# kolyangg/open-universe

Measured on AMD Instinct MI355X. Metric: sec-audio enhanced/sec/GPU + xRT, UNIVERSE++ 16 kHz 8 s clips @1/2/4/8 GPU, higher is better.
Workload: dtype f32 (conv operands split into f16 hi/lo: 3 f16 MFMA passes, f32 accumulation)

## Files before the change

### include/ouhip.h

```cpp
#ifndef OUHIP_H
#define OUHIP_H

#include <stddef.h>
#include <stdint.h>

#ifdef __cplusplus
extern "C" {
#endif

#define OUHIP_ABI_VERSION 10

int ou_abi_version(void);
const char* ou_last_error(void);

typedef struct ou_conv_desc {
    const float* x;
    int64_t x_bstride;
    int64_t x_cstride;
    int32_t cin;
    int32_t in_len;
    int32_t frame;
    int32_t shift;
    const float* in_scale;
    float slope;
    const float* w;
    int32_t m;
    int32_t kt;
    int32_t pad;
    int32_t cc;
    int32_t n_frames;
    int32_t batch;
    float* y;
    int64_t y_bstride, y_cstride;
    int32_t rout;
    int32_t out_len;
    int32_t valid_len;
    const float* bias;
    const float* res1;
    int64_t r1_bstride, r1_cstride;
    float s1;
    const float* film;
    int64_t film_bstride;
    const float* res2;
    int64_t r2_bstride, r2_cstride;
    float s2;
    int32_t tile;
    int32_t prec;
    float w_unscale;
    int32_t f0;
    int32_t* status;
    float* ks_ws;
    int64_t ks_ws_bytes;
    uint16_t* sy;
    int64_t sy_bstride;
    int32_t sy_rows;
    int32_t sy_shift;
    float sy_slope;
    int32_t sy_pad_;
    const uint16_t* xs;
    int64_t xs_bstride;
    int32_t xs_rows;
    int32_t xs_shift;
    int32_t fir;
    int32_t fir_pad_;
    const float* fir_taps;
} ou_conv_desc;

int ou_conv_chunk(int kt, int frame);
int64_t ou_conv_packed_size(int m, int cin_eff, int kt, int cc);
int ou_conv_pack(const float* w_logical, int m, int cin_eff, int kt, int cc,
                 float* packed);
int ou_conv_pack_split(const float* w_logical, int m, int cin_eff, int kt,
                       float* packed, float* w_unscale);
int ou_conv_pack_split_nat(const float* w_logical, int m, int cin_eff, int kt,
                           float* packed, float* w_unscale);
int ou_conv(const ou_conv_desc* d, void* stream);
int ou_conv_pick_tile(const ou_conv_desc* d);
int ou_conv_num_tiles(void);
int ou_conv_tile_ok(int kt, int tile);
int ou_conv_lds_info(int kt, int tile, int* lds_request, int* device_optin_max);

typedef struct ou_gru_desc {
    const float* gi;
    int64_t gi_bstride;
    const float* w_hh;
    const float* b_hh;
    float* y;
    int64_t y_bstride, y_cstride;
    const float* res;
    int64_t res_bstride, res_cstride;
    float res_scale;
    int32_t hidden;
    int32_t steps;
    int32_t batch;
    int32_t flags;
    uint64_t* granules;
    int32_t* status;
    int32_t t_begin, t_end;
    float* hstate;
    int32_t ws_zeroed;
    int32_t _pad;
} ou_gru_desc;

int64_t ou_gru_workspace_bytes(int hidden, int batch);
int ou_gru(const ou_gru_desc* d, void* stream);

typedef struct ou_embed_desc {
    const float* sigma;
    int32_t n;
    int32_t kind;
    int32_t dim;
    float te_weight, te_bias;
    const float* rff_freq;
    int32_t n_rff;
    int32_t rows;
    const float* mlp_w[3];
    const float* mlp_b[3];
    float mlp_slope[3];
    const float* w;
    const float* bias;
    float* out;
    float* gbuf;
} ou_embed_desc;

int ou_embed(const ou_embed_desc* d, void* stream);

typedef struct ou_head_desc {
    const float* h;
    int64_t h_bstride;
    int32_t channels, length, batch, mode;
    float slope1, slope2;
    const float* w;
    float bias;
    int32_t edm, _pad;
    float w_skip, w_out, s2, c_score, c_noise, s_next;
    const float* x;
    const float* z;
    float* out;
} ou_head_desc;

int ou_head(const ou_head_desc* d, void* stream);

int ou_normalize(const float* x, float* y, int batch, int64_t n, float level,
                 float eps, void* stream);
int ou_inv_rms(const float* x, float* out, int batch, int64_t n, float denom,
               float eps, void* stream);
int ou_rms(const float* x, float* out, int batch, int64_t n, void* stream);
int ou_power(const float* x, float* y, int batch, int nf, int frames, void* stream);
int ou_pad(const float* x, int64_t x_bstride, float* y, int batch, int n_in,
           int n_out, int left, void* stream);
int ou_scale(const float* z, float* y, int64_t n, float scale, const float* add,
             void* stream);
int ou_finish(const float* x, int64_t x_bstride, int left, float* y, int batch,
              int len, const float* mix_rms, void* stream);
int ou_ensemble_reduce(const float* x, float* y, int ensemble, int64_t n,
                       int mode , void* stream);
int ou_signal_median(const float* x, float* y, int ensemble, int batch, int64_t n, int* counts,
                     void* stream);

int ou_resample(const float* x, int64_t x_bstride, float* y, int64_t y_bstride, int batch, int n_in,
                int n_out, const float* kernel, int phases, int taps, int orig, int width, void* stream);

int ou_flac_info(const uint8_t* data, int64_t n, int32_t* sample_rate, int32_t* channels,
                 int32_t* bits_per_sample, int64_t* frames);
int64_t ou_flac_decode(const uint8_t* data, int64_t n, float* out, int64_t frames);
int64_t ou_flac_encode_bound(int channels, int64_t frames, int bps);
int64_t ou_flac_encode(const float* x, int channels, int64_t frames, int sample_rate, int bps, uint8_t* out,
                       int64_t capacity);

typedef struct ou_snake_desc {
    const float* h;
    int64_t h_bstride;
    int32_t channels, length, batch, _pad0;
    const float* alpha;
    const float* k_up;
    int32_t taps_up, width_up;
    const float* k_down;
    int32_t taps_down, width_down;
    float* out;
} ou_snake_desc;

int ou_snake_aa(const ou_snake_desc* d, void* stream);

typedef struct ou_block_desc {
    const float* h;
    int64_t h_bstride, h_cstride;
    int32_t channels, length;
    int32_t batch, prec;
    const void* w[3];
    const float* bias[3];
    float slope[3];
    float w_unscale[3];
    const float* sc;
    int64_t sc_bstride, sc_cstride;
    float s_sc;
    int32_t dbg;
    const float* film;
    int64_t film_bstride;
    float* cond_out;
    int64_t co_bstride, co_cstride;
    float* y;
    int64_t y_bstride, y_cstride;
    float s_res, s2;
    const float* res2;
    int64_t r2_bstride, r2_cstride;
    int32_t* status;
    const float* x;
    int64_t x_bstride;
    const float* in_scale;
    const float* w_in;
    const float* b_in;
    ou_head_desc head;
    const void* w_down;
    const float* b_down;
    float slope_down, w_down_unscale;
    int32_t rate, down_kt;
    float* e;
    int64_t e_bstride, e_cstride;
    int32_t f0, f1;
    int32_t h0, h1;
    int32_t shift[4];
    uint16_t* sy;
    int64_t sy_bstride;
    int32_t sy_rows, sy_shift;
    float sy_slope;
    int32_t sy_pad_;
    const uint16_t* xs;
    int64_t xs_bstride;
    int32_t xs_rows, xs_pad_;
} ou_block_desc;

int ou_block_supported(int channels, int prec);
int ou_block_frames(int channels);
int64_t ou_block_packed_halves(int channels, int kt);
int ou_block_pack(const float* w, int channels, int kt, void* out, float* w_unscale);
int ou_block_pack_rect(const float* w, int m, int channels, int kt, void* out, float* w_unscale);
int64_t ou_block_packed_f32(int channels, int kt);
int ou_block_pack_f32(const float* w, int channels, int kt, float* out, float* w_unscale);
int ou_block_down_supported(int channels, int rate, int kt, int prec);
int ou_block(const ou_block_desc* d, void* stream);

typedef struct ou_program ou_program;

enum {
    OU_OP_CONV = 1, OU_OP_GRU = 2, OU_OP_EMBED = 3, OU_OP_HEAD = 4,
    OU_OP_NORMALIZE = 5, OU_OP_INV_RMS = 6, OU_OP_POWER = 7, OU_OP_PAD = 8,
    OU_OP_SCALE = 9, OU_OP_FINISH = 10, OU_OP_RMS = 11, OU_OP_SNAKE = 12,
    OU_OP_MEMSET = 13, OU_OP_ENSEMBLE = 14, OU_OP_BLOCK = 15,
    OU_OP_LANE = 16, OU_OP_SIGNAL = 17, OU_OP_WAIT = 18
};

typedef struct ou_memset_desc {
    void* ptr;
    int64_t bytes;
} ou_memset_desc;
typedef struct ou_norm_args {
    const float* x;
// ... 123 lines not shown
```

### open_universe_amd/_lib.py

```python
import ctypes
import os
from ctypes import POINTER, c_char, c_char_p, c_float, c_int, c_int32, c_int64, c_size_t, c_uint32, c_uint64, c_void_p

_HERE = os.path.dirname(os.path.abspath(__file__))
LIB_PATH = os.environ.get("OUHIP_LIB", os.path.join(_HERE, "libouhip.so"))
ABI_VERSION = 10

fp = c_void_p

OP_CONV, OP_GRU, OP_EMBED, OP_HEAD = 1, 2, 3, 4
OP_NORMALIZE, OP_INV_RMS, OP_POWER, OP_PAD = 5, 6, 7, 8
OP_SCALE, OP_FINISH, OP_RMS, OP_SNAKE = 9, 10, 11, 12
OP_MEMSET, OP_ENSEMBLE, OP_BLOCK = 13, 14, 15
OP_LANE, OP_SIGNAL, OP_WAIT = 16, 17, 18


class ConvDesc(ctypes.Structure):
    _fields_ = [
        ("x", fp), ("x_bstride", c_int64), ("x_cstride", c_int64),
        ("cin", c_int32), ("in_len", c_int32), ("frame", c_int32), ("shift", c_int32),
        ("in_scale", fp), ("slope", c_float), ("w", fp),
        ("m", c_int32), ("kt", c_int32), ("pad", c_int32), ("cc", c_int32),
        ("n_frames", c_int32), ("batch", c_int32),
        ("y", fp), ("y_bstride", c_int64), ("y_cstride", c_int64),
# ... 3 lines not shown
        ("film", fp), ("film_bstride", c_int64),
        ("res2", fp), ("r2_bstride", c_int64), ("r2_cstride", c_int64), ("s2", c_float),
        ("tile", c_int32), ("prec", c_int32), ("w_unscale", c_float), ("f0", c_int32),
        ("status", fp), ("ks_ws", fp), ("ks_ws_bytes", c_int64),
        ("sy", fp), ("sy_bstride", c_int64), ("sy_rows", c_int32), ("sy_shift", c_int32),
        ("sy_slope", c_float), ("sy_pad_", c_int32),
        ("xs", fp), ("xs_bstride", c_int64), ("xs_rows", c_int32), ("xs_shift", c_int32),
        ("fir", c_int32), ("fir_pad_", c_int32), ("fir_taps", fp),
    ]


class GruDesc(ctypes.Structure):
    _fields_ = [
        ("gi", fp), ("gi_bstride", c_int64), ("w_hh", fp), ("b_hh", fp),
        ("y", fp), ("y_bstride", c_int64), ("y_cstride", c_int64),
        ("res", fp), ("res_bstride", c_int64), ("res_cstride", c_int64),
        ("res_scale", c_float), ("hidden", c_int32), ("steps", c_int32), ("batch", c_int32),
        ("flags", c_int32), ("granules", fp), ("status", fp), ("t_begin", c_int32), ("t_end", c_int32),
        ("hstate", fp), ("ws_zeroed", c_int32), ("_pad", c_int32),
    ]


class EmbedDesc(ctypes.Structure):
    _fields_ = [
        ("sigma", fp), ("n", c_int32), ("kind", c_int32), ("dim", c_int32),
        ("te_weight", c_float), ("te_bias", c_float), ("rff_freq", fp), ("n_rff", c_int32),
        ("rows", c_int32), ("mlp_w", fp * 3), ("mlp_b", fp * 3), ("mlp_slope", c_float * 3),
        ("w", fp), ("bias", fp), ("out", fp), ("gbuf", fp),
    ]


class HeadDesc(ctypes.Structure):
    _fields_ = [
        ("h", fp), ("h_bstride", c_int64),
        ("channels", c_int32), ("length", c_int32), ("batch", c_int32), ("mode", c_int32),
        ("slope1", c_float), ("slope2", c_float), ("w", fp), ("bias", c_float),
        ("edm", c_int32), ("_pad", c_int32),
        ("w_skip", c_float), ("w_out", c_float), ("s2", c_float), ("c_score", c_float),
        ("c_noise", c_float), ("s_next", c_float),
        ("x", fp), ("z", fp), ("out", fp),
    ]


class SnakeDesc(ctypes.Structure):
    _fields_ = [
        ("h", fp), ("h_bstride", c_int64),
        ("channels", c_int32), ("length", c_int32), ("batch", c_int32), ("_pad0", c_int32),
        ("alpha", fp), ("k_up", fp), ("taps_up", c_int32), ("width_up", c_int32),
        ("k_down", fp), ("taps_down", c_int32), ("width_down", c_int32), ("out", fp),
    ]


class SyncArgs(ctypes.Structure):
    _fields_ = [("id", c_int32), ("_pad", c_int32)]


class MemsetArgs(ctypes.Structure):
    _fields_ = [("ptr", fp), ("bytes", c_int64)]


class NormArgs(ctypes.Structure):
    _fields_ = [("x", fp), ("y", fp), ("batch", c_int32), ("_pad", c_int32), ("n", c_int64),
                ("level", c_float), ("eps", c_float)]


class RmsArgs(ctypes.Structure):
    _fields_ = [("x", fp), ("out", fp), ("batch", c_int32), ("_pad", c_int32), ("n", c_int64),
                ("denom", c_float), ("eps", c_float)]


class PowerArgs(ctypes.Structure):
    _fields_ = [("x", fp), ("y", fp), ("batch", c_int32), ("nf", c_int32),
                ("frames", c_int32), ("_pad", c_int32)]


class PadArgs(ctypes.Structure):
    _fields_ = [("x", fp), ("x_bstride", c_int64), ("y", fp), ("batch", c_int32),
                ("n_in", c_int32), ("n_out", c_int32), ("left", c_int32)]


class ScaleArgs(ctypes.Structure):
    _fields_ = [("z", fp), ("y", fp), ("n", c_int64), ("scale", c_float), ("_pad", c_float),
                ("add", fp)]


class FinishArgs(ctypes.Structure):
    _fields_ = [("x", fp), ("x_bstride", c_int64), ("left", c_int32), ("batch", c_int32),
                ("len", c_int32), ("_pad", c_int32), ("y", fp), ("mix_rms", fp)]


class EnsembleArgs(ctypes.Structure):
    _fields_ = [("x", fp), ("y", fp), ("ensemble", c_int32), ("mode", c_int32), ("n", c_int64),
                ("batch", c_int32), ("_pad", c_int32), ("counts", c_void_p)]


class BlockDesc(ctypes.Structure):
    _fields_ = [
        ("h", fp), ("h_bstride", c_int64), ("h_cstride", c_int64),
        ("channels", c_int32), ("length", c_int32), ("batch", c_int32), ("prec", c_int32),
        ("w", fp * 3), ("bias", fp * 3), ("slope", c_float * 3), ("w_unscale", c_float * 3),
        ("sc", fp), ("sc_bstride", c_int64), ("sc_cstride", c_int64), ("s_sc", c_float), ("dbg", c_int32),
        ("film", fp), ("film_bstride", c_int64),
        ("cond_out", fp), ("co_bstride", c_int64), ("co_cstride", c_int64),
        ("y", fp), ("y_bstride", c_int64), ("y_cstride", c_int64), ("s_res", c_float), ("s2", c_float),
        ("res2", fp), ("r2_bstride", c_int64), ("r2_cstride", c_int64),
        ("status", fp),
        ("x", fp), ("x_bstride", c_int64), ("in_scale", fp), ("w_in", fp), ("b_in", fp),
        ("head", HeadDesc),
        ("w_down", fp), ("b_down", fp), ("slope_down", c_float), ("w_down_unscale", c_float),
        ("rate", c_int32), ("down_kt", c_int32), ("e", fp), ("e_bstride", c_int64), ("e_cstride", c_int64),
        ("f0", c_int32), ("f1", c_int32), ("h0", c_int32), ("h1", c_int32),
        ("shift", c_int32 * 4),
        ("sy", fp), ("sy_bstride", c_int64), ("sy_rows", c_int32), ("sy_shift", c_int32),
        ("sy_slope", c_float), ("sy_pad_", c_int32),
        ("xs", fp), ("xs_bstride", c_int64), ("xs_rows", c_int32), ("xs_pad_", c_int32),
    ]


class BundleIo(ctypes.Structure):
    _fields_ = [("region", c_int32), ("count", c_int32), ("offset", c_int64),
                ("batch", c_int32), ("length", c_int32)]


class BundleMeta(ctypes.Structure):
    _fields_ = [("mix", BundleIo), ("noise", BundleIo), ("out", BundleIo), ("status", BundleIo),
                ("n_regions", c_int32), ("n_ops", c_int32), ("region_bytes", c_int64),
                ("json", c_char_p), ("json_bytes", c_int64), ("arch", c_char * 16)]


OP_STRUCT = {
    OP_CONV: ConvDesc, OP_GRU: GruDesc, OP_EMBED: EmbedDesc, OP_HEAD: HeadDesc,
    OP_NORMALIZE: NormArgs, OP_INV_RMS: RmsArgs, OP_RMS: RmsArgs, OP_POWER: PowerArgs,
    OP_PAD: PadArgs, OP_SCALE: ScaleArgs, OP_FINISH: FinishArgs, OP_SNAKE: SnakeDesc,
    OP_MEMSET: MemsetArgs, OP_ENSEMBLE: EnsembleArgs, OP_BLOCK: BlockDesc,
    OP_LANE: SyncArgs, OP_SIGNAL: SyncArgs, OP_WAIT: SyncArgs,
}

EXPORTS = {
    "ou_abi_version": (c_int, []),
    "ou_last_error": (ctypes.c_char_p, []),
    "ou_conv_chunk": (c_int, [c_int, c_int]),
    "ou_conv_packed_size": (c_int64, [c_int, c_int, c_int, c_int]),
    "ou_conv_pack": (c_int, [POINTER(c_float), c_int, c_int, c_int, c_int, POINTER(c_float)]),
    "ou_conv_pack_split": (c_int, [POINTER(c_float), c_int, c_int, c_int, POINTER(c_float),
                                   POINTER(c_float)]),
    "ou_conv_pack_split_nat": (c_int, [POINTER(c_float), c_int, c_int, c_int, POINTER(c_float),
                                       POINTER(c_float)]),
    "ou_conv": (c_int, [POINTER(ConvDesc), c_void_p]),
    "ou_conv_pick_tile": (c_int, [POINTER(ConvDesc)]),
    "ou_conv_num_tiles": (c_int, []),
    "ou_conv_tile_ok": (c_int, [c_int, c_int]),
    "ou_conv_lds_info": (c_int, [c_int, c_int, POINTER(c_int), POINTER(c_int)]),
    "ou_gru_workspace_bytes": (c_int64, [c_int, c_int]),
    "ou_gru": (c_int, [POINTER(GruDesc), c_void_p]),
    "ou_embed": (c_int, [POINTER(EmbedDesc), c_void_p]),
    "ou_head": (c_int, [POINTER(HeadDesc), c_void_p]),
    "ou_normalize": (c_int, [fp, fp, c_int, c_int64, c_float, c_float, c_void_p]),
    "ou_inv_rms": (c_int, [fp, fp, c_int, c_int64, c_float, c_float, c_void_p]),
    "ou_rms": (c_int, [fp, fp, c_int, c_int64, c_void_p]),
    "ou_power": (c_int, [fp, fp, c_int, c_int, c_int, c_void_p]),
    "ou_pad": (c_int, [fp, c_int64, fp, c_int, c_int, c_int, c_int, c_void_p]),
    "ou_scale": (c_int, [fp, fp, c_int64, c_float, fp, c_void_p]),
    "ou_finish": (c_int, [fp, c_int64, c_int, fp, c_int, c_int, fp, c_void_p]),
    "ou_ensemble_reduce": (c_int, [fp, fp, c_int, c_int64, c_int, c_void_p]),
    "ou_signal_median": (c_int, [fp, fp, c_int, c_int, c_int64, c_void_p, c_void_p]),
    "ou_snake_aa": (c_int, [POINTER(SnakeDesc), c_void_p]),
    "ou_block_supported": (c_int, [c_int, c_int]),
    "ou_block_frames": (c_int, [c_int]),
    "ou_block_packed_halves": (c_int64, [c_int, c_int]),
    "ou_block_pack": (c_int, [POINTER(c_float), c_int, c_int, c_void_p, POINTER(c_float)]),
    "ou_block_packed_f32": (c_int64, [c_int, c_int]),
    "ou_block_pack_f32": (c_int, [POINTER(c_float), c_int, c_int, POINTER(c_float), POINTER(c_float)]),
    "ou_block_pack_rect": (c_int, [POINTER(c_float), c_int, c_int, c_int, c_void_p, POINTER(c_float)]),
    "ou_block_down_supported": (c_int, [c_int, c_int, c_int, c_int]),
    "ou_block": (c_int, [POINTER(BlockDesc), c_void_p]),
    "ou_resample": (c_int, [fp, c_int64, fp, c_int64, c_int, c_int, c_int, fp, c_int, c_int, c_int, c_int,
                            c_void_p]),
    "ou_flac_info": (c_int, [c_void_p, c_int64, POINTER(c_int32), POINTER(c_int32), POINTER(c_int32),
                             POINTER(c_int64)]),
    "ou_flac_decode": (c_int64, [c_void_p, c_int64, c_void_p, c_int64]),
    "ou_flac_encode_bound": (c_int64, [c_int, c_int64, c_int]),
    "ou_flac_encode": (c_int64, [c_void_p, c_int, c_int64, c_int, c_int, c_void_p, c_int64]),
    "ou_program_create": (c_void_p, []),
    "ou_program_destroy": (None, [c_void_p]),
    "ou_program_add": (c_int, [c_void_p, c_int, c_void_p, c_size_t]),
    "ou_program_patch": (c_int, [c_void_p, c_int, c_int, c_void_p, c_size_t]),
    "ou_program_size": (c_int, [c_void_p]),
    "ou_program_run": (c_int, [c_void_p, c_void_p]),
    "ou_program_capture": (c_int, [c_void_p]),
    "ou_program_capture_segments": (c_int, [c_void_p]),
    "ou_program_validate": (c_int, [c_void_p]),
    "ou_program_launch": (c_int, [c_void_p, c_void_p]),
    "ou_program_op_kind": (c_int, [c_void_p, c_int]),
    "ou_program_profile": (c_int, [c_void_p, c_void_p, POINTER(c_float)]),
    "ou_program_trace": (c_int, [c_void_p, c_void_p, POINTER(c_float), POINTER(c_float)]),
    "ou_randn": (c_int, [fp, c_int64, c_uint64, c_uint64, c_void_p]),
    "ou_philox4x32": (c_int, [POINTER(c_uint32), POINTER(c_uint32), POINTER(c_uint32)]),
    "ou_bundle_open": (c_int, [c_char_p, POINTER(c_void_p)]),
    "ou_bundle_close": (None, [c_void_p]),
    "ou_bundle_info": (c_int, [c_void_p, POINTER(BundleMeta)]),
    "ou_bundle_region": (c_int, [c_void_p, c_int, POINTER(c_int32), POINTER(c_int64), POINTER(c_void_p)]),
    "ou_bundle_op": (c_int, [c_void_p, c_int, POINTER(c_int32), POINTER(c_int64), POINTER(c_char_p)]),
    "ou_bundle_materialize": (c_int, [c_void_p, POINTER(c_uint64), c_int, c_void_p]),
    "ou_bundle_load": (c_int, [c_char_p, c_int, POINTER(c_void_p)]),
    "ou_model_enhance_noise": (c_int, [c_void_p, fp, fp, fp, c_void_p]),
    "ou_model_enhance": (c_int, [c_void_p, fp, fp, c_uint64, c_uint64, c_void_p]),
    "ou_model_status": (c_int, [c_void_p]),
    "ou_model_info": (c_int, [c_void_p, POINTER(BundleMeta)]),
    "ou_model_destroy": (None, [c_void_p]),
    "ou_long_windows": (c_int, [c_int64, c_int, c_int, POINTER(c_int64), POINTER(c_int64)]),
    "ou_long_fade": (c_int, [c_int, POINTER(c_float)]),
    "ou_window_gather": (c_int, [fp, c_int64, c_int, c_int64, c_int, c_int, c_int64, c_int, c_int64, fp, c_int64,
                                 c_int64, c_void_p]),
    "ou_overlap_add": (c_int, [fp, c_int64, c_int64, c_int, c_int, c_int64, c_int, fp, fp, c_void_p]),
    "ou_model_long_noise": (c_int64, [c_void_p, c_int64, c_int, POINTER(c_int64)]),
    "ou_model_enhance_long_noise": (c_int, [c_void_p, fp, c_int64, c_int, fp, fp, c_void_p]),
    "ou_model_enhance_long": (c_int, [c_void_p, fp, c_int64, c_int, fp, c_uint64, c_uint64, fp, c_void_p]),
}

_lib = None


class OuHipError(RuntimeError):
    pass


class OuRangeError(OuHipError):
    flags = ()


def load():
    global _lib
    if _lib is not None:
        return _lib
    if not os.path.exists(LIB_PATH):
        raise OuHipError(
            f"{LIB_PATH} not found: build it with `python -c 'import __graft_entry__ as g; "
            "g.build()'` or open_universe_amd/csrc/build.sh")
    lib = ctypes.CDLL(LIB_PATH)
    for name, (res, args) in EXPORTS.items():
        f = getattr(lib, name)
        f.restype = res
        f.argtypes = args
    if lib.ou_abi_version() != ABI_VERSION:
        raise OuHipError("libouhip ABI version mismatch")
    _lib = lib
    return lib


def check(rc, what=""):
    if rc != 0:
        msg = load().ou_last_error()
        raise OuHipError(f"{what}: ouhip error {rc}: {msg.decode() if msg else ''}")


def conv_chunk(kt, frame):
    return load().ou_conv_chunk(kt, frame)


def conv_pack(w_logical, cc):
    import numpy as np

    w = np.ascontiguousarray(w_logical, dtype=np.float32)
    m, cin, kt = w.shape
    n = load().ou_conv_packed_size(m, cin, kt, cc)
    out = np.empty(n, dtype=np.float32)
    check(load().ou_conv_pack(w.ctypes.data_as(POINTER(c_float)), m, cin, kt, cc,
                              out.ctypes.data_as(POINTER(c_float))), "conv_pack")
    return out


def _split_scale(w):
    import numpy as np

    if not np.isfinite(w).all():
        raise OuHipError("split packing: non-finite weight")
    mx = float(np.abs(w).max()) if w.size else 0.0
    e = 0
    if mx > 0.0:
        e = min(100, max(-100, 10 - int(np.frexp(np.float32(mx))[1])))
    return np.float32(2.0**e), float(2.0 ** (6 - e))


def _hi_lo(a):
    import numpy as np

    hi = a.astype(np.float16)
    lo = ((a - hi.astype(np.float32)) * np.float32(2048.0)).astype(np.float16)
    return hi, lo


def conv_pack_split_np(w_logical):
    import numpy as np

    w = np.ascontiguousarray(w_logical, dtype=np.float32)
    m, cin, kt = w.shape
    sc, unscale = _split_scale(w)
    mt = (m + 31) // 32
    cpad = (cin + 63) // 64 * 64
    a = np.zeros((mt * 32, cpad, kt), dtype=np.float32)
    a[:m, :cin] = w * sc
    a = a.reshape(mt, 32, cpad // 16, 8, 2, kt).transpose(0, 2, 5, 4, 1, 3)
    hi, lo = _hi_lo(np.ascontiguousarray(a))
    out = np.stack([hi, lo], axis=2)
    return np.ascontiguousarray(out).reshape(-1).view(np.float32), unscale

# ... 218 lines not shown
```

### open_universe_amd/csrc/ou_gru.hip

```cpp
#include <hip/hip_runtime.h>

#include "../../include/ouhip.h"
#include "ou_common.h"

namespace {

constexpr int kMaxBatchPerWG = 4;

__host__ __device__ constexpr int64_t xcc_slot_base(int batch, int hidden) { return (int64_t)batch * 4 * hidden; }
__host__ __device__ constexpr int64_t xcc_slot_count(int batch, int hidden) { return (int64_t)batch * hidden / 4; }

#ifdef OU_GRU_STAMPS
constexpr int kStampSlots = 8;
#define OU_STAMP_INIT uint64_t st_[5] = {0, 0, 0, 0, 0}; uint64_t tp_ = __builtin_amdgcn_s_memtime();
#define OU_STAMP(i) do { const uint64_t n_ = __builtin_amdgcn_s_memtime(); st_[i] += n_ - tp_; tp_ = n_; } while (0)
#else
constexpr int kStampSlots = 0;
#define OU_STAMP_INIT
#define OU_STAMP(i) do { } while (0)
#endif

__device__ __forceinline__ float sigmoidf_(float x) { return 1.0f / (1.0f + expf(-x)); }

#define OU_DPP(v, ctrl) __builtin_bit_cast(float, __builtin_amdgcn_mov_dpp(__builtin_bit_cast(int, (v)), (ctrl), 0xF, 0xF, true))
__device__ __forceinline__ float sum8(float v)
{
    v += OU_DPP(v, 0xB1);
    v += OU_DPP(v, 0x4E);
    v += OU_DPP(v, 0x141);
    return v;
}

template <int H, int NB, int U>
__global__ __launch_bounds__(8 * U) void gru_kernel(ou_gru_desc d, int nb, int nchains, int flags)
{
    constexpr int G = H / U;
    constexpr int NT = 8 * U;
    constexpr int KPL = H / 8;
    constexpr int SEG = KPL + 4;
    __shared__ __attribute__((aligned(16))) float hs[NB][8 * SEG];
    __shared__ int abort_flag;

    const int bid = blockIdx.x;
    int chain, member;
    if (flags & 1) {
        const int c8 = bid & 7, rest = bid >> 3;
        member = rest % G;
        chain = (rest / G) * 8 + ((c8 - (flags >> 12)) & 7);
    } else {
        chain = bid / G;
        member = bid % G;
    }
    if (chain >= nchains) return;
    const int dir = chain & 1;
    const int b0 = (chain >> 1) * nb;

    const int tid = threadIdx.x;
    const int lane = tid & 63;
    const int wave = tid >> 6;
    const int kg = lane & 7;
    const int u = lane >> 3;
    const int j = member * U + wave * 8 + u;
    const int nbh = min(nb, d.batch - b0);
    const int T = d.steps;
    const bool sleep_poll = !(flags & 2);
    const bool nowait = flags & 16;
    if (tid == 0) abort_flag = 0;

    const float* wbase = d.w_hh + (int64_t)dir * 3 * H * H;
    float wr[KPL], wz[KPL], wn[KPL];
#pragma unroll
    for (int k = 0; k < KPL; k += 4) {
        const float4 a = *(const float4*)(wbase + (int64_t)(0 * H + j) * H + kg * KPL + k);
        const float4 bq = *(const float4*)(wbase + (int64_t)(1 * H + j) * H + kg * KPL + k);
        const float4 c = *(const float4*)(wbase + (int64_t)(2 * H + j) * H + kg * KPL + k);
        wr[k] = a.x; wr[k + 1] = a.y; wr[k + 2] = a.z; wr[k + 3] = a.w;
        wz[k] = bq.x; wz[k + 1] = bq.y; wz[k + 2] = bq.z; wz[k + 3] = bq.w;
        wn[k] = c.x; wn[k + 1] = c.y; wn[k + 2] = c.z; wn[k + 3] = c.w;
    }
    const float bhr = d.b_hh[dir * 3 * H + 0 * H + j];
    const float bhz = d.b_hh[dir * 3 * H + 1 * H + j];
    const float bhn = d.b_hh[dir * 3 * H + 2 * H + j];

    uint64_t* gran = d.granules;
    auto gidx = [&](int b, int par, int k) -> int64_t {
        return (((int64_t)b * 2 + dir) * 2 + par) * H + k;
    };

    float gir[NB], giz[NB], gin[NB], rsd[NB];
    auto prefetch = [&](int step, float* pr, float* pz, float* pn, float* pres) {
        const int tm = dir == 0 ? step : T - 1 - step;
#pragma unroll
        for (int bb = 0; bb < NB; ++bb) {
            if (bb < nbh && kg == 0) {
                const float* g = d.gi + (int64_t)(b0 + bb) * d.gi_bstride +
                                 (int64_t)(dir * 3 * H) * T + tm;
                pr[bb] = g[(int64_t)(0 * H + j) * T];
                pz[bb] = g[(int64_t)(1 * H + j) * T];
                pn[bb] = g[(int64_t)(2 * H + j) * T];
                pres[bb] = d.res ? d.res[(int64_t)(b0 + bb) * d.res_bstride +
                                         (int64_t)(dir * H + j) * d.res_cstride + tm]
                                 : 0.f;
            }
        }
    };
    prefetch(0, gir, giz, gin, rsd);
    OU_STAMP_INIT

    for (int t = 0; t < T; ++t) {
        const int time = dir == 0 ? t : T - 1 - t;
        if (t == 0) {
            for (int i = tid; i < nbh * H; i += NT) {
                const int bb = i / H, k = i - bb * H;
                hs[bb][(k / KPL) * SEG + (k % KPL)] = 0.f;
            }
        } else {
            const uint32_t want = (uint32_t)t;
            const int par = (t - 1) & 1;
            constexpr int NPER = (NB * H + NT - 1) / NT;
            uint64_t v[NPER];
            uint64_t* pp[NPER];
#pragma unroll
            for (int e = 0; e < NPER; ++e) {
                const int i = tid + e * NT;
                const int bb = i / H, k = i - bb * H;
                pp[e] = gran + gidx(b0 + min(bb, nbh - 1), par, k);
                v[e] = (i < nbh * H) ? __hip_atomic_load(pp[e], __ATOMIC_RELAXED, __HIP_MEMORY_SCOPE_AGENT)
                                     : ((uint64_t)want << 32);
            }
            uint32_t spins = 0;
            while (true) {
                bool ok = true;
                if (nowait) break;
#pragma unroll
                for (int e = 0; e < NPER; ++e) ok &= (uint32_t)(v[e] >> 32) == want;
                if (ok) break;
                if (sleep_poll) __builtin_amdgcn_s_sleep(1);
                if (++spins > (1u << 23)) {
                    atomicExch(d.status, 1);
                    abort_flag = 1;
                    break;
                }
#pragma unroll
                for (int e = 0; e < NPER; ++e)
                    if ((uint32_t)(v[e] >> 32) != want)
                        v[e] = __hip_atomic_load(pp[e], __ATOMIC_RELAXED, __HIP_MEMORY_SCOPE_AGENT);
            }
            OU_STAMP(0);
#pragma unroll
            for (int e = 0; e < NPER; ++e) {
                const int i = tid + e * NT;
                if (i < nbh * H) {
                    const int bb = i / H, k = i - bb * H;
                    hs[bb][(k / KPL) * SEG + (k % KPL)] = __uint_as_float((uint32_t)v[e]);
                }
            }
        }
        __syncthreads();
        if (abort_flag) return;
        OU_STAMP(1);

        float cr[NB], cz[NB], cn[NB], cres[NB];
#pragma unroll
        for (int bb = 0; bb < NB; ++bb) {
            cr[bb] = gir[bb]; cz[bb] = giz[bb]; cn[bb] = gin[bb]; cres[bb] = rsd[bb];
        }
        if (t + 1 < T) prefetch(t + 1, gir, giz, gin, rsd);

#pragma unroll
        for (int bb = 0; bb < NB; ++bb) {
            if (bb >= nbh) break;
            const float* hv = &hs[bb][kg * SEG];
            float sr = 0.f, sz = 0.f, sn = 0.f;
#pragma unroll
            for (int k = 0; k < KPL; k += 4) {
                const float4 hq = *(const float4*)(hv + k);
                sr = fmaf(wr[k], hq.x, sr); sz = fmaf(wz[k], hq.x, sz); sn = fmaf(wn[k], hq.x, sn);
                sr = fmaf(wr[k + 1], hq.y, sr); sz = fmaf(wz[k + 1], hq.y, sz); sn = fmaf(wn[k + 1], hq.y, sn);
                sr = fmaf(wr[k + 2], hq.z, sr); sz = fmaf(wz[k + 2], hq.z, sz); sn = fmaf(wn[k + 2], hq.z, sn);
                sr = fmaf(wr[k + 3], hq.w, sr); sz = fmaf(wz[k + 3], hq.w, sz); sn = fmaf(wn[k + 3], hq.w, sn);
            }
            sr = sum8(sr);
            sz = sum8(sz);
            sn = sum8(sn);
            OU_STAMP(2);
            if (kg == 0) {
                const float hprev = hs[bb][(j / KPL) * SEG + (j % KPL)];
                const float r = sigmoidf_(cr[bb] + (sr + bhr));
                const float z = sigmoidf_(cz[bb] + (sz + bhz));
                const float n = tanhf(cn[bb] + r * (sn + bhn));
                const float hn = (1.0f - z) * n + z * hprev;
                const int b = b0 + bb;
                if (t + 1 < T) {
                    const uint64_t g = ((uint64_t)(uint32_t)(t + 1) << 32) | __float_as_uint(hn);
                    __hip_atomic_store(gran + gidx(b, t & 1, j), g, __ATOMIC_RELAXED,
                                       __HIP_MEMORY_SCOPE_AGENT);
                }
                const int64_t c = (int64_t)(dir * H + j);
                const float out = d.res ? (hn + cres[bb]) * d.res_scale : hn;
                d.y[(int64_t)b * d.y_bstride + c * d.y_cstride + time] = out;
            }
        }
        OU_STAMP(3);
        __syncthreads();
        OU_STAMP(4);
    }
#ifdef OU_GRU_STAMPS
    if (tid == 0) {
        uint64_t* o = gran + xcc_slot_base(d.batch, H) + xcc_slot_count(d.batch, H) + (int64_t)bid * kStampSlots;
        for (int i = 0; i < 5; ++i) o[i] = st_[i];
        o[5] = T;
    }
#endif
}


__device__ __forceinline__ float fast_sigmoid(float x)
{
    return __builtin_amdgcn_rcpf(1.0f + __builtin_amdgcn_exp2f(-1.44269504088896341f * x));
}
__device__ __forceinline__ float fast_tanh(float x)
{
    return fmaf(2.0f, fast_sigmoid(2.0f * x), -1.0f);
}

__device__ __forceinline__ void swap32(float& x, float& y)
{
    const auto r = __builtin_amdgcn_permlane32_swap(__float_as_uint(x), __float_as_uint(y), false, false);
    x = __uint_as_float(r[0]);
    y = __uint_as_float(r[1]);
}
__device__ __forceinline__ void swap16(float& x, float& y)
{
    const auto r = __builtin_amdgcn_permlane16_swap(__float_as_uint(x), __float_as_uint(y), false, false);
    x = __uint_as_float(r[0]);
    y = __uint_as_float(r[1]);
}

constexpr int kKsWaves = 4;


template <int H, int NB, int UW>
__global__ __launch_bounds__(64 * kKsWaves) void gru_ks_kernel(ou_gru_desc d, int nb, int nchains, int flags,
                                                               int bofs)
{
    constexpr int KPL = H / 64;
    constexpr int G = H / (UW * kKsWaves);
    constexpr int NV = UW * 3 * NB;
    constexpr int NG = 3 * NB;
    constexpr int USH = UW == 8 ? 3 : 4;
    static_assert(H % 64 == 0 && G >= 1 && (UW == 4 || UW == 8), "k-split GRU: H % 64 == 0, UW 4 or 8");

    const int bid = blockIdx.x;
    int chain, member;
    if (flags & 1) {
        const int c8 = bid & 7, rest = bid >> 3;
        member = rest % G;
        chain = (rest / G) * 8 + ((c8 - (flags >> 12)) & 7);
    } else {
        chain = bid / G;
        member = bid % G;
    }
    if (chain >= nchains) return;
    const int dir = chain & 1;
    const int b0 = bofs + (chain >> 1) * nb;
    const int nbh = min(nb, d.batch - b0);
    const int T = d.steps;
    const bool sleep_poll = !(flags & 2);

    const int lane = threadIdx.x & 63;
    const int wave = threadIdx.x >> 6;
    const int ubase = (member * kKsWaves + wave) * UW;
    const int j = ubase + (lane >> USH);
    const bool writer = (lane & ((1 << USH) - 1)) == 0;

    float w[UW][3][KPL];
    const float* wbase = d.w_hh + (int64_t)dir * 3 * H * H + lane * KPL;
#pragma unroll
    for (int u = 0; u < UW; ++u)
#pragma unroll
        for (int g = 0; g < 3; ++g)
#pragma unroll
            for (int k = 0; k < KPL; ++k) w[u][g][k] = wbase[(int64_t)(g * H + ubase + u) * H + k];
    const float bhr = d.b_hh[dir * 3 * H + 0 * H + j];
    const float bhz = d.b_hh[dir * 3 * H + 1 * H + j];
    const float bhn = d.b_hh[dir * 3 * H + 2 * H + j];

    uint64_t* gran = d.granules;

    bool local_l2 = false;
    if (!(flags & 64)) {
        uint32_t xcc;
        asm volatile("s_getreg_b32 %0, hwreg(HW_REG_XCC_ID, 0, 4)" : "=s"(xcc));
        uint64_t* xs = gran + xcc_slot_base(d.batch, H) + ((int64_t)b0 * 2 + dir) * G;
        if (threadIdx.x == 0)
            __hip_atomic_store(xs + member, (1ull << 32) | xcc, __ATOMIC_RELAXED, __HIP_MEMORY_SCOPE_AGENT);
        uint64_t v = 0;
        for (uint32_t spins = 0;; ++spins) {
            v = lane < G ? __hip_atomic_load(xs + lane, __ATOMIC_RELAXED, __HIP_MEMORY_SCOPE_AGENT)
                         : ((1ull << 32) | xcc);
            if (__all((uint32_t)(v >> 32) == 1u)) break;
            if (spins > (1u << 23)) {
                if (lane == 0) atomicExch(d.status, 1);
                return;
            }
            __builtin_amdgcn_s_sleep(1);
        }
        local_l2 = __all((uint32_t)v == xcc);
    }
    const int64_t gran_bytes = (int64_t)d.batch * 2 * 2 * H * 8;
    const __amdgpu_buffer_rsrc_t grsrc =
        ou_rsrc(gran, gran_bytes);
    auto goff = [&](int b, int par) -> int {
        return (int)(((((int64_t)b * 2 + dir) * 2 + par) * H + lane * KPL) * 8);
    };

    const int tb = d.t_begin, te = d.t_end > 0 ? min(d.t_end, T) : T;
    float hp[NB];
    float gir[NB], giz[NB], gin[NB], rsd[NB];
    auto prefetch = [&](int step) {
        const int tm = dir == 0 ? step : T - 1 - step;
#pragma unroll
        for (int bb = 0; bb < NB; ++bb) {
            if (bb < nbh) {
                const float* g = d.gi + (int64_t)(b0 + bb) * d.gi_bstride + (int64_t)(dir * 3 * H) * T + tm;
                gir[bb] = g[(int64_t)(0 * H + j) * T];
                giz[bb] = g[(int64_t)(1 * H + j) * T];
                gin[bb] = g[(int64_t)(2 * H + j) * T];
                rsd[bb] = d.res ? d.res[(int64_t)(b0 + bb) * d.res_bstride +
                                        (int64_t)(dir * H + j) * d.res_cstride + tm]
                                : 0.f;
            }
        }
    };
    constexpr int CS = UW == 4 ? 128 : 64;
    const bool stage = NB == 1 && !(flags & 256);
    float4* gst = nullptr;
    if constexpr (NB == 1) {
        __shared__ float4 gst_all[kKsWaves][CS * UW];
        gst = gst_all[wave];
    }
    const int wv = __builtin_amdgcn_readfirstlane(wave);
    auto stage_chunk = [&](int c0) {
        constexpr int NV4 = 4 * UW * CS / 64;
        const int ub = (member * kKsWaves + wv) * UW;
        float v[NV4];
#pragma unroll
        for (int i = 0; i < NV4; ++i) {
            const int e = lane + 64 * i, row = e / CS, st = min(c0 + e % CS, te - 1);
            const int tm = dir == 0 ? st : T - 1 - st;
            if (row < 3 * UW) {
                const int g = row / UW, u = row % UW;
                v[i] = d.gi[(int64_t)b0 * d.gi_bstride + (int64_t)(dir * 3 * H + g * H + ub + u) * T + tm];
            } else {
                const int u = row - 3 * UW;
                v[i] = d.res ? d.res[(int64_t)b0 * d.res_bstride + (int64_t)(dir * H + ub + u) * d.res_cstride + tm]
                             : 0.f;
            }
        }
#pragma unroll
        for (int i = 0; i < NV4; ++i) {
            const int e = lane + 64 * i, row = e / CS, sc = e % CS;
            const int comp = row < 3 * UW ? row / UW : 3, u = row < 3 * UW ? row % UW : row - 3 * UW;
            ((float*)gst)[(sc * UW + u) * 4 + comp] = v[i];
        }
    };
    auto hs_at = [&](int b, int u) -> float {
        return tb > 0 ? d.hstate[((int64_t)b * 2 + dir) * H + u] : 0.f;
    };
    float h0[NB][KPL];
#pragma unroll
    for (int bb = 0; bb < NB; ++bb) {
        hp[bb] = hs_at(b0 + min(bb, nbh - 1), j);
#pragma unroll
        for (int k = 0; k < KPL; ++k) h0[bb][k] = hs_at(b0 + min(bb, nbh - 1), lane * KPL + k);
    }
    if (stage) stage_chunk(tb);
    else prefetch(tb);
    OU_STAMP_INIT

    for (int t = tb; t < te; ++t) {
        const int time = dir == 0 ? t : T - 1 - t;
        float h[NB][KPL];
        float4 gv{};
        if (stage) {
            if (t > tb && (t - tb) % CS == 0) stage_chunk(t);
            gv = gst[((t - tb) % CS) * UW + (lane >> USH)];
        }
        if (t == tb) {
#pragma unroll
            for (int bb = 0; bb < NB; ++bb)
#pragma unroll
                for (int k = 0; k < KPL; ++k) h[bb][k] = h0[bb][k];
        } else {
            const uint32_t want = (uint32_t)t;
            const int par = (t - 1) & 1;
            for (uint32_t spins = 0;; ++spins) {
                bool ok = true;
#pragma unroll
                for (int bb = 0; bb < NB; ++bb) {
                    const int b = b0 + min(bb, nbh - 1);
                    if constexpr (KPL % 2 == 0) {
#pragma unroll
                        for (int q = 0; q < KPL / 2; ++q) {
                            const auto v = __builtin_amdgcn_raw_buffer_load_b128(grsrc, goff(b, par) + 16 * q, 0, 16);
                            h[bb][2 * q] = __uint_as_float(v[0]);
                            h[bb][2 * q + 1] = __uint_as_float(v[2]);
                            ok &= bb >= nbh || (v[1] == want && v[3] == want);
                        }
                    } else {
#pragma unroll
                        for (int k = 0; k < KPL; ++k) {
                            const uint64_t v = __hip_atomic_load(
                                gran + ((((int64_t)b * 2 + dir) * 2 + par) * H + lane * KPL + k),
                                __ATOMIC_RELAXED, __HIP_MEMORY_SCOPE_AGENT);
                            h[bb][k] = __uint_as_float((uint32_t)v);
                            ok &= bb >= nbh || (uint32_t)(v >> 32) == want;
                        }
                    }
                }
                if (__all(ok)) break;
                if (sleep_poll) __builtin_amdgcn_s_sleep(1);
                if (spins > (1u << 23)) {
                    if (lane == 0) atomicExch(d.status, 1);
                    return;
                }
                asm volatile("" ::: "memory");
            }
        }
        OU_STAMP(0);

        float cr[NB], cz[NB], cn[NB], cres[NB];
        if (stage) {
            cr[0] = gv.x, cz[0] = gv.y, cn[0] = gv.z, cres[0] = gv.w;
        } else {
#pragma unroll
            for (int bb = 0; bb < NB; ++bb) {
                cr[bb] = gir[bb]; cz[bb] = giz[bb]; cn[bb] = gin[bb]; cres[bb] = rsd[bb];
            }
            if (t + 1 < te) prefetch(t + 1);
        }

        float acc[NV];
#pragma unroll
        for (int u = 0; u < UW; ++u)
#pragma unroll
            for (int bb = 0; bb < NB; ++bb)
#pragma unroll
                for (int g = 0; g < 3; ++g) {
                    float a = 0.f;
#pragma unroll
                    for (int k = 0; k < KPL; ++k) a = fmaf(w[u][g][k], h[bb][k], a);
                    acc[(u * NB + bb) * 3 + g] = a;
                }
        OU_STAMP(1);

#pragma unroll
        for (int i = 0; i < NV / 2; ++i) {
            swap32(acc[i], acc[i + NV / 2]);
            acc[i] += acc[i + NV / 2];
        }
#pragma unroll
        for (int i = 0; i < NV / 4; ++i) {
            swap16(acc[i], acc[i + NV / 4]);
            acc[i] += acc[i + NV / 4];
        }
        if constexpr (UW == 8) {
            const bool hi8 = lane & 8;
#pragma unroll
            for (int i = 0; i < NG; ++i) {
                const float send = hi8 ? acc[i] : acc[i + NG];
                const float keep = hi8 ? acc[i + NG] : acc[i];
                acc[i] = keep + OU_DPP(send, 0x128);
            }
        } else {
#pragma unroll
            for (int i = 0; i < NG; ++i) acc[i] += OU_DPP(acc[i], 0x128);
        }
#pragma unroll
        for (int i = 0; i < NG; ++i) acc[i] = sum8(acc[i]);
        OU_STAMP(2);

#pragma unroll
        for (int bb = 0; bb < NB; ++bb) {
            if (bb >= nbh) break;
            const float r = fast_sigmoid(cr[bb] + (acc[bb * 3 + 0] + bhr));
            const float z = fast_sigmoid(cz[bb] + (acc[bb * 3 + 1] + bhz));
            const float n = fast_tanh(cn[bb] + r * (acc[bb * 3 + 2] + bhn));
            const float hn = (1.0f - z) * n + z * hp[bb];
            hp[bb] = hn;
            if (writer) {
                const int b = b0 + bb;
                if (t + 1 < T) {
                    const uint64_t gv = ((uint64_t)(uint32_t)(t + 1) << 32) | __float_as_uint(hn);
                    uint64_t* gp = gran + ((((int64_t)b * 2 + dir) * 2 + (t & 1)) * H + j);
                    if (local_l2)
                        __hip_atomic_store(gp, gv, __ATOMIC_RELAXED, __HIP_MEMORY_SCOPE_WORKGROUP);
                    else
                        __hip_atomic_store(gp, gv, __ATOMIC_RELAXED, __HIP_MEMORY_SCOPE_AGENT);
                }
                const float out = d.res ? (hn + cres[bb]) * d.res_scale : hn;
                d.y[(int64_t)b * d.y_bstride + (int64_t)(dir * H + j) * d.y_cstride + time] = out;
            }
        }
        OU_STAMP(3);
    }
    if (d.hstate && writer) {
#pragma unroll
        for (int bb = 0; bb < NB; ++bb)
            if (bb < nbh) d.hstate[((int64_t)(b0 + bb) * 2 + dir) * H + j] = hp[bb];
    }
    if (!(flags & 64) && threadIdx.x == 0)
        __hip_atomic_store(gran + xcc_slot_base(d.batch, H) + ((int64_t)b0 * 2 + dir) * G + member, (uint64_t)0,
                           __ATOMIC_RELAXED, __HIP_MEMORY_SCOPE_AGENT);
#ifdef OU_GRU_STAMPS
    if (lane == 0 && wave == 0) {
        uint64_t* o = gran + xcc_slot_base(d.batch, H) + xcc_slot_count(d.batch, H) + (int64_t)bid * kStampSlots;
        for (int i = 0; i < 4; ++i) o[i] = st_[i];
        o[4] = local_l2;
        o[5] = T;
    }
#endif
}

template <int H, int NB, int UW>
void launch_ks(const ou_gru_desc& d, int nb, int nchains, int flags, int bofs, hipStream_t s)
{
    constexpr int G = H / (UW * kKsWaves);
    const int grid = (flags & 1) ? 8 * G * ((nchains + 7) / 8) : nchains * G;
    hipLaunchKernelGGL((gru_ks_kernel<H, NB, UW>), dim3(grid), dim3(64 * kKsWaves), 0, s, d, nb, nchains, flags,
                       bofs);
}

constexpr int kKsMaxWGs = 256;

template <int H, int UW>
int launch_ks_uw(const ou_gru_desc& d, int flags, hipStream_t s)
{
    constexpr int G = H / (UW * kKsWaves);
    constexpr int kMaxNb = H >= 512 ? 2 : 4;
    int nb = 1;
    while (nb < kMaxNb && 2 * ((d.batch + nb - 1) / nb) * G > kKsMaxWGs) nb *= 2;
    const int per_launch = (kKsMaxWGs / (2 * G)) * nb;
    for (int b = 0; b < d.batch; b += per_launch) {
        const int items = min(per_launch, d.batch - b);
        const int nchains = 2 * ((items + nb - 1) / nb);
        if (nb == 1) launch_ks<H, 1, UW>(d, nb, nchains, flags, b, s);
        else if (nb == 2 || kMaxNb == 2) launch_ks<H, 2, UW>(d, nb, nchains, flags, b, s);
        else launch_ks<H, kMaxNb, UW>(d, nb, nchains, flags, b, s);
    }
    return 0;
}

template <int H>
int launch_ks_all(const ou_gru_desc& d, int flags, hipStream_t s)
{
    constexpr int G4 = H / (4 * kKsWaves);
    if (!(flags & 128) && 2 * d.batch * G4 <= kKsMaxWGs) return launch_ks_uw<H, 4>(d, flags, s);
    return launch_ks_uw<H, 8>(d, flags, s);
}

template <int H, int NB, int U>
void launch_u(const ou_gru_desc& d, int nb, int nchains, int flags, hipStream_t s)
{
    constexpr int G = H / U;
    const int grid = (flags & 1) ? 8 * G * ((nchains + 7) / 8) : nchains * G;
    hipLaunchKernelGGL((gru_kernel<H, NB, U>), dim3(grid), dim3(8 * U), 0, s, d, nb, nchains, flags);
}

template <int H, int NB>
void launch_nb(const ou_gru_desc& d, int nb, int nchains, int flags, hipStream_t s)
{
    if ((flags & 8) && H >= 128 && H % 128 == 0)
        launch_u<H, NB, (H >= 128 ? 128 : 32)>(d, nb, nchains, flags, s);
    else if ((flags & 4) && H >= 64 && H % 64 == 0)
        launch_u<H, NB, (H >= 64 ? 64 : 32)>(d, nb, nchains, flags, s);
    else
        launch_u<H, NB, 32>(d, nb, nchains, flags, s);
}

template <int H>
void launch_h(const ou_gru_desc& d, int nb, int nchains, int flags, hipStream_t s)
{
    if (nb == 1) launch_nb<H, 1>(d, nb, nchains, flags, s);
    else if (nb == 2) launch_nb<H, 2>(d, nb, nchains, flags, s);
    else launch_nb<H, 4>(d, nb, nchains, flags, s);
}

}

extern "C" int64_t ou_gru_workspace_bytes(int hidden, int batch)
{
    return (xcc_slot_base(batch, hidden) + xcc_slot_count(batch, hidden) + (int64_t)kStampSlots * 1024) *
           (int64_t)sizeof(uint64_t);
}

static int gru_after(const ou_gru_desc& d, hipStream_t s)
{
    const int rc = ou_check_launch("gru");
    if (rc == 0 && d.ws_zeroed && d.steps < 5)
        OU_HIP_CHECK(hipMemsetAsync(d.granules, 0, ou_gru_workspace_bytes(d.hidden, d.batch), s), "gru: memset");
    return rc;
}

extern "C" int ou_gru(const ou_gru_desc* dp, void* stream)
{
    if (!dp) return ou_fail(-1, "gru: null descriptor");
    const ou_gru_desc& d = *dp;
    if (!d.gi || !d.b_hh || !d.y || d.steps <= 0 || d.batch <= 0 || d.batch > 32768)
        return ou_fail(-1, "gru: invalid descriptor");
    hipStream_t s = (hipStream_t)stream;
    const bool split = d.t_begin != 0 || (d.t_end != 0 && d.t_end != d.steps);
    const bool dflt = d.flags < 0 || (d.flags & 0x8000);
    const int fbits = dflt ? -1 : (d.flags & 0xfff), fofs = d.flags >= 0 ? (d.flags & 0x7000) : 0;
    if (d.t_begin < 0 || (d.t_end != 0 && (d.t_end <= d.t_begin || d.t_end > d.steps)) || (split && !d.hstate))
        return ou_fail(-1, "gru: bad step range [%d, %d) of %d (hstate %p)", d.t_begin, d.t_end, d.steps,
                       (const void*)d.hstate);
    if (split && (d.hidden % 64 || (fbits >= 0 && (fbits & 32))))
        return ou_fail(-2, "gru: a step range needs the k-split kernel (hidden %% 64 == 0)");
    if (!d.w_hh || !d.granules || !d.status) return ou_fail(-1, "gru: invalid descriptor");
    if ((!d.ws_zeroed && d.t_begin == 0) || d.steps < 5)
        OU_HIP_CHECK(hipMemsetAsync(d.granules, 0, ou_gru_workspace_bytes(d.hidden, d.batch), s), "gru: memset");
    if (d.hidden % 64 == 0 && !(fbits >= 0 && (fbits & 32))) {
        const int kflags = (fbits >= 0 ? fbits : 1) | fofs;
        switch (d.hidden) {
        case 64: launch_ks_all<64>(d, kflags, s); break;
        case 128: launch_ks_all<128>(d, kflags, s); break;
        case 256: launch_ks_all<256>(d, kflags, s); break;
        case 384: launch_ks_all<384>(d, kflags, s); break;
        case 512: launch_ks_all<512>(d, kflags, s); break;
        default: return ou_fail(-1, "gru: unsupported hidden size %d", d.hidden);
        }
        return gru_after(d, s);
    }
    const int nb = d.batch >= kMaxBatchPerWG ? kMaxBatchPerWG : (d.batch >= 2 ? 2 : 1);
    const int nchains = 2 * ((d.batch + nb - 1) / nb);
    const int flags = (fbits >= 0 ? fbits : (nb == 1 ? 5 : 1)) | fofs;
    if (nchains * (d.hidden / 32) > 512) return ou_fail(-2, "gru: grid too large for residency");
    switch (d.hidden) {
    case 32: launch_h<32>(d, nb, nchains, flags, s); break;
    case 64: launch_h<64>(d, nb, nchains, flags, s); break;
    case 128: launch_h<128>(d, nb, nchains, flags, s); break;
    case 256: launch_h<256>(d, nb, nchains, flags, s); break;
    case 384: launch_h<384>(d, nb, nchains, flags, s); break;
    default: return ou_fail(-1, "gru: unsupported hidden size %d", d.hidden);
    }
    return gru_after(d, s);
}
```

Measured before the change: 761.6.

## Add straight-line specialized k-split GRU step loop with packed f32x2 FMA

After: 796.9 (median of 6 runs). 4.6% higher.

```diff
diff --git a/include/ouhip.h b/include/ouhip.h
--- a/include/ouhip.h
+++ b/include/ouhip.h
@@ -103,6 +103,7 @@
 } ou_gru_desc;
 
 int64_t ou_gru_workspace_bytes(int hidden, int batch);
+int ou_gru_ks_max_workgroups(void);
 int ou_gru(const ou_gru_desc* d, void* stream);
 
 typedef struct ou_embed_desc {
diff --git a/open_universe_amd/_lib.py b/open_universe_amd/_lib.py
--- a/open_universe_amd/_lib.py
+++ b/open_universe_amd/_lib.py
@@ -179,6 +179,7 @@
     "ou_conv_tile_ok": (c_int, [c_int, c_int]),
     "ou_conv_lds_info": (c_int, [c_int, c_int, POINTER(c_int), POINTER(c_int)]),
     "ou_gru_workspace_bytes": (c_int64, [c_int, c_int]),
+    "ou_gru_ks_max_workgroups": (c_int, []),
     "ou_gru": (c_int, [POINTER(GruDesc), c_void_p]),
     "ou_embed": (c_int, [POINTER(EmbedDesc), c_void_p]),
     "ou_head": (c_int, [POINTER(HeadDesc), c_void_p]),
diff --git a/open_universe_amd/csrc/ou_gru.hip b/open_universe_amd/csrc/ou_gru.hip
--- a/open_universe_amd/csrc/ou_gru.hip
+++ b/open_universe_amd/csrc/ou_gru.hip
@@ -1,4 +1,6 @@
 #include <hip/hip_runtime.h>
+
+#include <type_traits>
 
 #include "../../include/ouhip.h"
 #include "ou_common.h"
@@ -237,10 +239,33 @@
     y = __uint_as_float(r[1]);
 }
 
+typedef float f32x2 __attribute__((ext_vector_type(2)));
+template <int N>
+__device__ __forceinline__ void add_halves(float* acc)
+{
+    if constexpr (N % 2 == 0) {
+#pragma unroll
+        for (int i = 0; i < N; i += 2) {
+            const f32x2 s = (f32x2){acc[i], acc[i + 1]} + (f32x2){acc[i + N], acc[i + N + 1]};
+            acc[i] = s.x;
+            acc[i + 1] = s.y;
+        }
+    } else {
+#pragma unroll
+        for (int i = 0; i < N; ++i) acc[i] += acc[i + N];
+    }
+}
+
+__device__ __forceinline__ float blend_nofma(float z, float n, float hp)
+{
+#pragma clang fp contract(off)
+    return (1.0f - z) * n + z * hp;
+}
+
 constexpr int kKsWaves = 4;
 
 
-template <int H, int NB, int UW>
+template <int H, int NB, int UW, bool LEGACY>
 __global__ __launch_bounds__(64 * kKsWaves) void gru_ks_kernel(ou_gru_desc d, int nb, int nchains, int flags,
                                                                int bofs)
 {
@@ -282,6 +307,14 @@
         for (int g = 0; g < 3; ++g)
 #pragma unroll
             for (int k = 0; k < KPL; ++k) w[u][g][k] = wbase[(int64_t)(g * H + ubase + u) * H + k];
+    f32x2 wp[NB == 1 && !LEGACY ? NV / 2 : 1][KPL];
+    if constexpr (NB == 1 && !LEGACY) {
+#pragma unroll
+        for (int p = 0; p < NV / 2; ++p)
+#pragma unroll
+            for (int k = 0; k < KPL; ++k)
+                wp[p][k] = (f32x2){w[(2 * p) / 3][(2 * p) % 3][k], w[(2 * p + 1) / 3][(2 * p + 1) % 3][k]};
+    }
     const float bhr = d.b_hh[dir * 3 * H + 0 * H + j];
     const float bhz = d.b_hh[dir * 3 * H + 1 * H + j];
     const float bhn = d.b_hh[dir * 3 * H + 2 * H + j];
@@ -334,14 +367,14 @@
         }
     };
     constexpr int CS = UW == 4 ? 128 : 64;
-    const bool stage = NB == 1 && !(flags & 256);
+    const bool stage = NB == 1 && (!LEGACY || !(flags & 256));
     float4* gst = nullptr;
     if constexpr (NB == 1) {
         __shared__ float4 gst_all[kKsWaves][CS * UW];
         gst = gst_all[wave];
     }
     const int wv = __builtin_amdgcn_readfirstlane(wave);
-    auto stage_chunk = [&](int c0) {
+    auto stage_chunk = [&](int c0) __attribute__((always_inline)) {
         constexpr int NV4 = 4 * UW * CS / 64;
         const int ub = (member * kKsWaves + wv) * UW;
         float v[NV4];
@@ -379,6 +412,135 @@
     else prefetch(tb);
     OU_STAMP_INIT
 
+    if constexpr (!LEGACY) {
+        static_assert(NB == 1, "the straight-line loop carries one item per chain");
+        auto run = [&](auto local_c, auto res_c) __attribute__((always_inline)) -> bool {
+            constexpr bool LOCAL = decltype(local_c)::value, RES = decltype(res_c)::value;
+            const float res_scale = d.res_scale;
+            float* yrow = d.y + (int64_t)b0 * d.y_bstride + (int64_t)(dir * H + j) * d.y_cstride;
+            uint64_t* gpub = gran + (((int64_t)b0 * 2 + dir) * 2) * H + j;
+            auto poll = [&](int t, float (&h)[KPL]) __attribute__((always_inline)) -> bool {
+                const uint32_t want = (uint32_t)t;
+                const int par = (t - 1) & 1;
+                for (uint32_t spins = 0;; ++spins) {
+                    bool ok = true;
+                    if constexpr (KPL % 2 == 0) {
+#pragma unroll
+                        for (int q = 0; q < KPL / 2; ++q) {
+                            const auto v = __builtin_amdgcn_raw_buffer_load_b128(grsrc, goff(b0, par) + 16 * q, 0, 16);
+                            h[2 * q] = __uint_as_float(v[0]);
+                            h[2 * q + 1] = __uint_as_float(v[2]);
+                            ok &= v[1] == want && v[3] == want;
+                        }
+                    } else {
+#pragma unroll
+                        for (int k = 0; k < KPL; ++k) {
+                            const uint64_t v = __hip_atomic_load(
+                                gran + ((((int64_t)b0 * 2 + dir) * 2 + par) * H + lane * KPL + k),
+                                __ATOMIC_RELAXED, __HIP_MEMORY_SCOPE_AGENT);
+                            h[k] = __uint_as_float((uint32_t)v);
+                            ok &= (uint32_t)(v >> 32) == want;
+                        }
+                    }
+                    if (__all(ok)) return true;
+                    __builtin_amdgcn_s_sleep(1);
+                    if (spins > (1u << 23)) {
+                        if (lane == 0) atomicExch(d.status, 1);
+                        return false;
+                    }
+                    asm volatile("" ::: "memory");
+                }
+            };
+            auto step = [&](int t, int sc, auto first_c, auto pub_c) __attribute__((always_inline)) -> bool {
+                constexpr bool FIRST = decltype(first_c)::value, PUB = decltype(pub_c)::value;
+                float h[KPL];
+                const float4 gv = gst[sc * UW + (lane >> USH)];
+                if constexpr (FIRST) {
+#pragma unroll
+                    for (int k = 0; k < KPL; ++k) h[k] = h0[0][k];
+                } else {
+                    if (!poll(t, h)) return false;
+                }
+                OU_STAMP(0);
+
+                float acc[NV];
+#pragma unroll
+                for (int p = 0; p < NV / 2; ++p) {
+                    f32x2 a = {0.f, 0.f};
+#pragma unroll
+                    for (int k = 0; k < KPL; ++k) a = __builtin_elementwise_fma(wp[p][k], (f32x2){h[k], h[k]}, a);
+                    acc[2 * p] = a.x;
+                    acc[2 * p + 1] = a.y;
+                }
+                OU_STAMP(1);
+
+#pragma unroll
+                for (int i = 0; i < NV / 2; ++i) swap32(acc[i], acc[i + NV / 2]);
+                add_halves<NV / 2>(acc);
+#pragma unroll
+                for (int i = 0; i < NV / 4; ++i) swap16(acc[i], acc[i + NV / 4]);
+                add_halves<NV / 4>(acc);
+                if constexpr (UW == 8) {
+                    const bool hi8 = lane & 8;
+#pragma unroll
+                    for (int i = 0; i < NG; ++i) {
+                        const float send = hi8 ? acc[i] : acc[i + NG];
+                        const float keep = hi8 ? acc[i + NG] : acc[i];
+                        acc[i] = keep + OU_DPP(send, 0x128);
+                    }
+                } else {
+#pragma unroll
+                    for (int i = 0; i < NG; ++i) acc[i] += OU_DPP(acc[i], 0x128);
+                }
+#pragma unroll
+                for (int i = 0; i < NG; ++i) acc[i] = sum8(acc[i]);
+                OU_STAMP(2);
+
+                const float r = fast_sigmoid(gv.x + (acc[0] + bhr));
+                const float z = fast_sigmoid(gv.y + (acc[1] + bhz));
+                const float n = fast_tanh(gv.z + r * (acc[2] + bhn));
+                const float hn = blend_nofma(z, n, hp[0]);
+                if constexpr (PUB) {
+                    if (writer) {
+                        const uint64_t gw = ((uint64_t)(uint32_t)(t + 1) << 32) | __float_as_uint(hn);
+                        uint64_t* gp = gpub + (t & 1) * H;
+                        if constexpr (LOCAL)
+                            __hip_atomic_store(gp, gw, __ATOMIC_RELAXED, __HIP_MEMORY_SCOPE_WORKGROUP);
+                        else
+                            __hip_atomic_store(gp, gw, __ATOMIC_RELAXED, __HIP_MEMORY_SCOPE_AGENT);
+                    }
+                }
+                hp[0] = hn;
+                if (writer) yrow[dir == 0 ? t : T - 1 - t] = RES ? (hn + gv.w) * res_scale : hn;
+                OU_STAMP(3);
+                return true;
+            };
+            constexpr std::true_type yes{};
+            constexpr std::false_type no{};
+            const int tmid = min(te, T - 1);
+            if (tb < tmid) {
+                if (!step(tb, 0, yes, yes)) return false;
+            } else {
+                if (!step(tb, 0, yes, no)) return false;
+            }
+            int sc = 1;
+            for (int t = tb + 1; t < tmid; ++t) {
+                if (!step(t, sc, no, yes)) return false;
+                if (++sc == CS && t + 1 < te) {
+                    stage_chunk(t + 1);
+                    sc = 0;
+                }
+            }
+            if (te == T && T - 1 > tb) {
+                if (!step(T - 1, sc, no, no)) return false;
+            }
+            return true;
+        };
+        bool done;
+        if (local_l2) done = d.res ? run(std::true_type{}, std::true_type{}) : run(std::true_type{}, std::false_type{});
+        else done = d.res ? run(std::false_type{}, std::true_type{}) : run(std::false_type{}, std::false_type{});
+        if (!done) return;
+    } else
     for (int t = tb; t < te; ++t) {
         const int time = dir == 0 ? t : T - 1 - t;
         float h[NB][KPL];
@@ -528,8 +690,12 @@
 {
     constexpr int G = H / (UW * kKsWaves);
     const int grid = (flags & 1) ? 8 * G * ((nchains + 7) / 8) : nchains * G;
-    hipLaunchKernelGGL((gru_ks_kernel<H, NB, UW>), dim3(grid), dim3(64 * kKsWaves), 0, s, d, nb, nchains, flags,
-                       bofs);
+    if (NB > 1 || (flags & (512 | 256 | 2)))
+        hipLaunchKernelGGL((gru_ks_kernel<H, NB, UW, true>), dim3(grid), dim3(64 * kKsWaves), 0, s, d, nb, nchains,
+                           flags, bofs);
+    else if constexpr (NB == 1)
+        hipLaunchKernelGGL((gru_ks_kernel<H, NB, UW, false>), dim3(grid), dim3(64 * kKsWaves), 0, s, d, nb, nchains,
+                           flags, bofs);
 }
 
 constexpr int kKsMaxWGs = 256;
@@ -594,6 +760,8 @@
     return (xcc_slot_base(batch, hidden) + xcc_slot_count(batch, hidden) + (int64_t)kStampSlots * 1024) *
            (int64_t)sizeof(uint64_t);
 }
+
+extern "C" int ou_gru_ks_max_workgroups(void) { return kKsMaxWGs; }
 
 static int gru_after(const ou_gru_desc& d, hipStream_t s)
 {
```
